# reuk/parallel-reverb-raytracer

Measured on AMD Instinct MI355X. Metric: ray_bounces_per_sec, higher is better.
Workload: dtype f32; 1 GPU; cathedral stand-in (Sibenik unavailable offline), 75252 triangles, 100000 rays/GPU x 128 bounces x 8 bands, 2 cardioid speakers, 44100 Hz, trim_predelay, output_mode all, histogram mode exact; triangles=75252, rays_per_gpu=100000, reflections=128, histogram_mode=exact: the reference's serial float sum over all impulses, bit for bit

## Files before the change

### parallel-reverb-raytracer_amd/csrc/ctx.h

```cpp
#pragma once

#include "../../include/rvb_capi.h"
#include "hip_owned.h"
#include "ir_state.h"
#include "kept_state.h"
#include "kernels.h"
#include "merged_state.h"
#include "source_state.h"
#include "trace_state.h"

#include <cmath>
#include <cstddef>
#include <cstring>
#include <memory>
#include <string>
#include <utility>
#include <vector>

#pragma GCC visibility push(hidden)

struct SceneStore {
    int device = 0;
    DevBuf nodes, tris, shade, corners, surfaces;
    ~SceneStore() { (void) hipSetDevice(device); }
// ... 350 lines not shown
    void end_timing(hipStream_t on = nullptr) { if (timing_open) (void) hipEventRecord(timings.back().stop, on ? on : stream.h); timing_open = false; }
    void reset_timings() { timings.clear(); events_used = 0; }
    void void_fetched_results() { trace.records_rewritten(); ir.drop_configuration(); }
    void void_trace() { trace.inputs_changed(); ir.drop_configuration(); merged.void_list(); }
};

int fail(rvb_ctx * ctx, int code, const std::string & what);
#define RVB_BIND(ctx) RVB_HIP(fail, ctx, hipSetDevice((ctx)->device))

inline const rvb_impulse * ir_diffuse(const rvb_ctx * ctx)
{
    return ctx->trace.impulses.as<rvb_impulse>() + ctx->trace.pair() * ctx->nrays * ctx->trace.nreflections();
}
struct IrCounts { uint64_t ndiffuse, nimages; };
inline IrCounts ir_counts(const rvb_ctx * ctx)
{
    return {(ctx->ir.which() & RVB_IR_DIFFUSE) ? ctx->nrays * ctx->trace.nreflections() : 0, (ctx->ir.which() & RVB_IR_IMAGES) ? ctx->ir.nimages() : 0};
}

inline uint64_t bins_for(float max_time, float predelay, float sample_rate)
{
    const float t = max_time > predelay ? max_time - predelay : 0.0f;
    return (uint64_t) (roundf(t * sample_rate) + 1);
}

inline int key_bits_for(uint64_t nbins)
{
    int bits = 1;
    while (bits < 32 && (1ull << bits) < nbins + 1)
        ++bits;
    return bits;
}

int fetch_small(rvb_ctx * ctx);
int reset_time_ranges(rvb_ctx * ctx, const TraceArgs & a);
int launch_images_beside(rvb_ctx * ctx, TraceArgs & a);
int launch_shadow_behind_images(rvb_ctx * ctx, const TraceArgs & a, const SourceShading & source, bool gains_stand = false);
int check_source_counts(rvb_ctx * ctx, const char * who, uint64_t npairs);
int apply_source_patterns(rvb_ctx * ctx, const TraceArgs & a, const SourceShading & source, bool gains_stand = false);
int download_surface_gradient(rvb_ctx * ctx, const float * d_out, rvb_surface * grad_surfaces, float grad_air[8]);

int merge_image_winners(const rvb_image_candidate * candidates, uint64_t ncandidates, bool have_direct, bool remove_direct, std::vector<uint32_t> & winners);
int ir_speaker_model(rvb_ctx * ctx, const float mic[3], const rvb_speaker * speakers, uint64_t nspeakers);
int ir_hrtf_model(rvb_ctx * ctx, const float mic[3], const float * table, const float facing[3], const float up[3]);
int ir_configure_refusals(rvb_ctx * ctx, int which);
int ir_configure_images(rvb_ctx * ctx, int which, const rvb_impulse * images, uint64_t nimages, bool gathered);
int ir_images_on_host(rvb_ctx * ctx);
int upload_hrtf_table(rvb_ctx * ctx, const float * table, int first_ear, int ears);
AttenuationModel hrtf_model(const rvb_ctx * ctx, const float mic[3], const float facing[3], const float up[3]);

bool own_sort_enabled();
int own_sort(rvb_ctx * ctx, const uint32_t * keys, uint32_t value_base, uint64_t n, int begin_bit, int end_bit,
             uint32_t * keys_out, uint32_t * values_out, bool want_keys);
int ensure_sort_buffers(rvb_ctx * ctx, uint64_t n);
int sort_and_bin(rvb_ctx * ctx, uint64_t n, uint64_t nkeys, int key_bits, bool may_sort_own);

#pragma GCC visibility pop
```

### parallel-reverb-raytracer_amd/csrc/exact_kernels.hip

```cpp
#include "attenuation.h"

#define SUM_UNROLL 4
#define RVB_HRTF_SUM_THREADS 256
#define WIDE_BINS 32
#define WIDE_MAX_WAVES 4

namespace {

__global__ __launch_bounds__(256) void bin_keys_kernel(ModelDev m, uint32_t ch, const rvb_impulse * __restrict__ in, uint64_t n,
                                                       uint64_t index_base, float predelay, float sample_rate, uint32_t sentinel,
                                                       uint32_t * __restrict__ keys, uint32_t * __restrict__ values)
{
    for (uint64_t i = (uint64_t) blockIdx.x * blockDim.x + threadIdx.x; i < n; i += (uint64_t) gridDim.x * blockDim.x) {
        const float4 * r = reinterpret_cast<const float4 *>(in + i);
        const float4 v0 = r[0], v1 = r[1], p = r[2];
        const float time = r[3].x;
        const bool nonzero = ANY_VOLUME(v0, v1);
        uint32_t key = sentinel;
        if (nonzero) key = min(time_bin(attenuated_time(m, ch, mk3(p.x, p.y, p.z), time), predelay, sample_rate), sentinel);
        keys[index_base + i] = key;
        values[index_base + i] = (uint32_t) (index_base + i);
    }
}

// ... 107 lines not shown
#pragma unroll 4
        for (uint32_t r = 0; r < LIVE_ROUNDS; ++r) {
            const uint64_t j = tile * RVB_LIVE_TILE + r * 64u + lane;
            const uint32_t key = j < n ? raw[j] : LIVE_DEAD;
            const bool live = key != LIVE_DEAD;
            const unsigned long long mask = __ballot(live);
            if (live) {
                const uint64_t to = at + lanes_below(mask);
                if (to < listed) {
                    keys[to] = key;
                    values[to] = (uint32_t) j;
                    if (HRTF) {
                        keys[listed + to] = raw[n + j];
                        values[listed + to] = (uint32_t) j;
                    }
                } else {
                    *overflow = 1u;
                }
            }
            at += (uint64_t) __popcll(mask);
        }
    }
    const uint64_t total = head->total < listed ? head->total : listed;
    for (uint64_t k = total + (uint64_t) blockIdx.x * blockDim.x + threadIdx.x; k < listed; k += (uint64_t) gridDim.x * blockDim.x) {
        keys[k] = nbins;
        values[k] = 0u;
        if (HRTF) {
            keys[listed + k] = 2u * nbins + 1u;
            values[listed + k] = 0u;
        }
    }
}

__global__ __launch_bounds__(256) void bin_starts_kernel(const uint32_t * __restrict__ keys, uint64_t n, uint64_t nbins, uint32_t * __restrict__ starts,
                                                         uint32_t * __restrict__ ends)
{
    for (uint64_t k = (uint64_t) blockIdx.x * blockDim.x + threadIdx.x; k < n; k += (uint64_t) gridDim.x * blockDim.x) {
        const uint32_t key = keys[k];
        if (key >= nbins)
            continue;
        if (k == 0 || keys[k - 1] != key)
            starts[key] = (uint32_t) k;
        if (k + 1 == n || keys[k + 1] != key)
            ends[key] = (uint32_t) (k + 1);
    }
}

template <bool HRTF, int NCH>
__global__ __launch_bounds__(64) void ordered_sum_kernel(ModelDev m, uint32_t first_channel, const rvb_impulse * __restrict__ diffuse,
                                                         uint64_t ndiffuse, const rvb_impulse * __restrict__ images,
                                                         const uint32_t * __restrict__ values,
                                                         const uint32_t * __restrict__ starts, const uint32_t * __restrict__ ends,
                                                         uint64_t nbins, uint64_t bin_begin, uint64_t bin_end, float * __restrict__ hist)
{
    const uint64_t t = (uint64_t) blockIdx.x * blockDim.x + threadIdx.x;
    const uint64_t bin = bin_begin + (t >> 1);
    const uint32_t half = (uint32_t) t & 1u;
    if (bin >= bin_end)
        return;
    const uint64_t lo = starts[bin];
    if (lo == 0xFFFFFFFFull)
        return;
    float sum[NCH][4];
#pragma unroll
    for (int c = 0; c < NCH; ++c)
#pragma unroll
        for (int b = 0; b < 4; ++b)
            sum[c][b] = hist[hist_row(first_channel + c, half, b, nbins) + bin];
    const uint64_t hi = ends[bin];
    for (uint64_t k = lo; k < hi; k += SUM_UNROLL) {
        float4 v[SUM_UNROLL], p[SUM_UNROLL];
        gather_records<SUM_UNROLL>(values, k, lo, hi, diffuse, ndiffuse, images, half, v, p);
#pragma unroll
        for (int u = 0; u < SUM_UNROLL; ++u) {
            if (k + u >= hi) break;
            const float vol[4] = {v[u].x, v[u].y, v[u].z, v[u].w};
            const v3 pos = mk3(p[u].x, p[u].y, p[u].z);
            if (HRTF) {
                const float * tb = m.table + ((uint64_t) first_channel * RVB_HRTF_ROWS + (uint64_t) hrtf_row(m, pos)) * 8 + half * 4;
#pragma unroll
                for (int b = 0; b < 4; ++b) sum[0][b] += vol[b] * tb[b];
            } else {
#pragma unroll
                for (int c = 0; c < NCH; ++c) {
                    const float g = speaker_gain(m, first_channel + c, pos);
#pragma unroll
                    for (int b = 0; b < 4; ++b) sum[c][b] += vol[b] * g;
                }
            }
        }
    }
#pragma unroll
    for (int c = 0; c < NCH; ++c)
#pragma unroll
        for (int b = 0; b < 4; ++b)
            hist[hist_row(first_channel + c, half, b, nbins) + bin] = sum[c][b];
}

__global__ __launch_bounds__(RVB_HRTF_SUM_THREADS) void ordered_sum_hrtf_kernel(ModelDev m, const rvb_impulse * __restrict__ diffuse, uint64_t ndiffuse,
                                                              const rvb_impulse * __restrict__ images, const uint32_t * __restrict__ values,
                                                              const uint32_t * __restrict__ starts, const uint32_t * __restrict__ ends,
                                                              uint64_t nbins, uint64_t bin_begin, uint64_t bin_end, float * __restrict__ hist)
{
    const uint64_t t = (uint64_t) blockIdx.x * blockDim.x + threadIdx.x;
    const uint64_t slot = 2 * bin_begin + (t >> 1);
    const uint32_t half = (uint32_t) t & 1u;
    if (slot >= 2 * bin_end)
        return;
    const uint32_t ear = (uint32_t) slot & 1u;
    const uint64_t bin = slot >> 1;
    const uint64_t key = (uint64_t) ear * (nbins + 1) + bin;
    const uint64_t lo = starts[key];
    if (lo == 0xFFFFFFFFull)
        return;
    float sum[4];
#pragma unroll
    for (int b = 0; b < 4; ++b)
        sum[b] = hist[((uint64_t) ear * 8 + half * 4 + b) * nbins + bin];
    const uint64_t hi = ends[key];
    const float * table = m.table + (uint64_t) ear * RVB_HRTF_ROWS * 8 + half * 4;
    for (uint64_t k = lo; k < hi; k += SUM_UNROLL) {
        float4 v[SUM_UNROLL], p[SUM_UNROLL];
        gather_records<SUM_UNROLL>(values, k, lo, hi, diffuse, ndiffuse, images, half, v, p);
#pragma unroll
        for (int u = 0; u < SUM_UNROLL; ++u) {
            if (k + u >= hi) break;
            const float4 tb = *reinterpret_cast<const float4 *>(table + (uint64_t) hrtf_row_quad(m, mk3(p[u].x, p[u].y, p[u].z), half) * 8);
            sum[0] += v[u].x * tb.x;
            sum[1] += v[u].y * tb.y;
// ... 100 lines not shown
        const float4 * r = reinterpret_cast<const float4 *>(in + values[k]);
        const float4 v0 = r[0], v1 = r[1];
        sum[0] += v0.x; sum[1] += v0.y; sum[2] += v0.z; sum[3] += v0.w;
        sum[4] += v1.x; sum[5] += v1.y; sum[6] += v1.z; sum[7] += v1.w;
    }
    for (int b = 0; b < 8; ++b)
        out[(uint64_t) b * nbins + bin] = sum[b];
}

bool fold_range(uint64_t nbins, uint64_t bin_begin, uint64_t & bin_end)
{
    bin_end = std::min(bin_end, nbins);
    return bin_begin < bin_end;
}

}

void rvb_launch_bin_keys(const AttenuationModel & m, uint32_t channel, const rvb_impulse * in, uint64_t n, uint64_t index_base,
                         float predelay, float sample_rate, uint32_t sentinel, uint32_t * keys, uint32_t * values, hipStream_t s)
{
    if (n == 0) return;
    hipLaunchKernelGGL(bin_keys_kernel, dim3(stream_blocks(n, 256)), dim3(256), 0, s, make_model(m), channel, in, n,
                       index_base, predelay, sample_rate, sentinel, keys, values);
}

void rvb_launch_bin_keys_hrtf(const AttenuationModel & m, const rvb_impulse * in, uint64_t count, uint64_t index_base, uint64_t n,
                              float predelay, float sample_rate, uint32_t nbins, uint32_t * keys, uint32_t * values, hipStream_t s)
{
    if (count == 0) return;
    hipLaunchKernelGGL(bin_keys_hrtf_kernel, dim3(stream_blocks(count, 256)), dim3(256), 0, s, make_model(m), in, count, index_base, n,
                       predelay, sample_rate, nbins, keys, values);
}

void rvb_launch_bin_starts(const uint32_t * sorted_keys, uint64_t n, uint64_t nbins, uint32_t * starts, uint32_t * ends, hipStream_t s)
{
    if (n == 0) return;
    hipLaunchKernelGGL(bin_starts_kernel, dim3(stream_blocks(n, 256)), dim3(256), 0, s, sorted_keys, n, nbins, starts, ends);
}

size_t rvb_live_scratch_bytes(uint64_t n)
{
    return sizeof(LiveHeader) + (size_t) ((n + RVB_LIVE_TILE - 1) / RVB_LIVE_TILE) * sizeof(uint32_t);
}

void rvb_launch_live_list(const AttenuationModel & m, const rvb_impulse * diffuse, uint64_t ndiffuse, const rvb_impulse * images, uint64_t n,
                          float predelay, float sample_rate, uint32_t nbins, uint64_t listed, uint32_t * raw, void * scratch,
                          uint32_t * keys, uint32_t * values, uint32_t * overflow, hipStream_t s)
{
    if (n == 0) return;
    LiveHeader * head = static_cast<LiveHeader *>(scratch);
    uint32_t * tiles = reinterpret_cast<uint32_t *>(head + 1);
    const uint64_t ntiles = (n + RVB_LIVE_TILE - 1) / RVB_LIVE_TILE;
    const dim3 grid(stream_blocks(ntiles, LIVE_WAVES)), block(64 * LIVE_WAVES);
    const ModelDev md = make_model(m);
    if (m.hrtf) {
        hipLaunchKernelGGL(live_keys_kernel<true>, grid, block, 0, s, md, diffuse, ndiffuse, images, n, predelay, sample_rate, nbins, raw, tiles);
        hipLaunchKernelGGL(live_offsets_kernel, dim3(1), dim3(LIVE_OFFSET_THREADS), 0, s, tiles, ntiles, head);
        hipLaunchKernelGGL(live_compact_kernel<true>, grid, block, 0, s, raw, n, tiles, head, listed, nbins, keys, values, overflow);
    } else {
        hipLaunchKernelGGL(live_keys_kernel<false>, grid, block, 0, s, md, diffuse, ndiffuse, images, n, predelay, sample_rate, nbins, raw, tiles);
        hipLaunchKernelGGL(live_offsets_kernel, dim3(1), dim3(LIVE_OFFSET_THREADS), 0, s, tiles, ntiles, head);
        hipLaunchKernelGGL(live_compact_kernel<false>, grid, block, 0, s, raw, n, tiles, head, listed, nbins, keys, values, overflow);
    }
}

void rvb_launch_ordered_sum(const AttenuationModel & m, uint32_t first_channel, uint32_t nchannels, const rvb_impulse * diffuse,
                            uint64_t ndiffuse, const rvb_impulse * images,
                            const uint32_t * sorted_values, const uint32_t * starts, const uint32_t * ends, uint64_t n,
                            uint64_t nbins, float * hist, hipStream_t s, uint64_t bin_begin, uint64_t bin_end)
{
    if (!fold_range(nbins, bin_begin, bin_end) || n == 0) return;
    const dim3 grid((unsigned) ((2 * (bin_end - bin_begin) + 63) / 64)), block(64);
    const ModelDev md = make_model(m);
#define RVB_SUM(HRTF, NCH) hipLaunchKernelGGL((ordered_sum_kernel<HRTF, NCH>), grid, block, 0, s, md, first_channel, diffuse, ndiffuse, \
                                              images, sorted_values, starts, ends, nbins, bin_begin, bin_end, hist)
    if (m.hrtf) { RVB_SUM(true, 1); return; }
    switch (nchannels) {
    case 1: RVB_SUM(false, 1); break;
    case 2: RVB_SUM(false, 2); break;
    case 3: RVB_SUM(false, 3); break;
    case 4: RVB_SUM(false, 4); break;
    default:
        for (uint32_t c = 0; c < nchannels; c += 4) {
            const uint32_t k = nchannels - c < 4 ? nchannels - c : 4;
            rvb_launch_ordered_sum(m, first_channel + c, k, diffuse, ndiffuse, images, sorted_values, starts, ends, n, nbins, hist, s, bin_begin, bin_end);
        }
    }
#undef RVB_SUM
}

void rvb_launch_ordered_sum_hrtf(const AttenuationModel & m, const rvb_impulse * diffuse, uint64_t ndiffuse, const rvb_impulse * images,
                                 const uint32_t * sorted_values, const uint32_t * starts, const uint32_t * ends, uint64_t nbins, float * hist,
                                 hipStream_t s, uint64_t bin_begin, uint64_t bin_end)
{
    if (!fold_range(nbins, bin_begin, bin_end)) return;
    const dim3 grid((unsigned) ((4 * (bin_end - bin_begin) + RVB_HRTF_SUM_THREADS - 1) / RVB_HRTF_SUM_THREADS));
    hipLaunchKernelGGL(ordered_sum_hrtf_kernel, grid, dim3(RVB_HRTF_SUM_THREADS), 0, s, make_model(m), diffuse, ndiffuse,
                       images, sorted_values, starts, ends, nbins, bin_begin, bin_end, hist);
}

void rvb_make_speaker_table(const rvb_speaker * speakers, uint64_t nspeakers, float4 * table)
{
    for (uint64_t i = 0; i < nspeakers; ++i)
        table[i] = speaker_device_form(speakers[i]);
}

void rvb_launch_ordered_sum_wide(const AttenuationModel & m, const rvb_impulse * diffuse, uint64_t ndiffuse, const rvb_impulse * images,
                                 const uint32_t * sorted_values, const uint32_t * starts, const uint32_t * ends, uint64_t n,
                                 uint64_t nbins, float * hist, hipStream_t s, uint64_t bin_begin, uint64_t bin_end)
{
    if (!fold_range(nbins, bin_begin, bin_end) || n == 0 || m.nchannels == 0 || !m.speaker_table) return;
    const uint32_t per_wave = wide_channels_per_wave(m.nchannels);
    const uint32_t waves = (m.nchannels + per_wave - 1) / per_wave;
    const dim3 grid((unsigned) ((bin_end - bin_begin + WIDE_BINS - 1) / WIDE_BINS)), block(64 * waves);
    const v3 mic = mk3(m.mic[0], m.mic[1], m.mic[2]);
    if (per_wave == 12)
        hipLaunchKernelGGL(ordered_sum_wide_kernel<12>, grid, block, 0, s, mic, m.speaker_table, m.nchannels, diffuse, ndiffuse, images,
                           sorted_values, starts, ends, nbins, bin_begin, bin_end, hist);
// ... 20 lines not shown
```

### parallel-reverb-raytracer_amd/csrc/ir.hip

```cpp
#include "bin_blocks.h"
#include "ctx.h"

#include <algorithm>
#include <cstdlib>
#include <cstring>

int upload_hrtf_table(rvb_ctx * ctx, const float * table, int first_ear, int ears)
{
    const size_t rows = RVB_HRTF_ROWS - 1;
    std::vector<float> padded((size_t) 2 * RVB_HRTF_ROWS * 8, 0.0f);
    for (int e = 0; e < ears; ++e)
        std::memcpy(padded.data() + (size_t) (first_ear + e) * RVB_HRTF_ROWS * 8, table + (size_t) e * rows * 8, rows * 8 * sizeof(float));
    RVB_HIP(fail, ctx, ctx->ir.hrtf_table.ensure(padded.size() * sizeof(float)));
    RVB_HIP(fail, ctx, hipMemcpy(ctx->ir.hrtf_table.p, padded.data(), padded.size() * sizeof(float), hipMemcpyHostToDevice));
    return RVB_OK;
}

AttenuationModel hrtf_model(const rvb_ctx * ctx, const float mic[3], const float facing[3], const float up[3])
{
    AttenuationModel m;
    m.hrtf = 1;
    m.nchannels = 2;
    m.hrtf_table = ctx->ir.hrtf_table.as<const float>();
    for (int i = 0; i < 3; ++i) { m.mic[i] = mic[i]; m.facing[i] = facing[i]; m.up[i] = up[i]; }
// ... 102 lines not shown
    in.ndiffuse = count.ndiffuse;
    in.nimages = count.nimages;
    in.n = in.ndiffuse + in.nimages;
    if (in.n >= (1ull << 31)) return fail(ctx, RVB_ERR_CAPACITY, "rvb_ir_accumulate: too many impulses for exact mode");
    if (nbins >= 0x7FFFFFF0ull) return fail(ctx, RVB_ERR_CAPACITY, "rvb_ir_accumulate: too many bins for exact mode");
    in.listed = in.n;
    return ensure_sort_buffers(ctx, lists * in.n);
}

int live_list(rvb_ctx * ctx, ExactList & in, float predelay, float sample_rate, uint64_t nbins)
{
    in.compacted = true;
    in.count_valid = ctx->trace.live_count_holds();
    if (in.count_valid && in.ndiffuse) {
        const int rc = fetch_small(ctx);
        if (rc != RVB_OK) return rc;
        in.listed = std::min<uint64_t>(ctx->trace.live_count(), in.ndiffuse) + in.nimages;
    }
    RVB_HIP(fail, ctx, ctx->sort.live.ensure(rvb_live_scratch_bytes(in.n)));
    rvb_launch_live_list(ctx->ir.model, ir_diffuse(ctx), in.ndiffuse, ctx->ir.images.as<rvb_impulse>(), in.n, predelay, sample_rate, (uint32_t) nbins,
                         in.listed, ctx->sort.keys_b.as<uint32_t>(), ctx->sort.live.p, ctx->sort.keys_a.as<uint32_t>(), ctx->sort.vals_a.as<uint32_t>(),
                         &ctx->trace.host->live_overflow, ctx->stream);
    return RVB_OK;
}

int exact_list(rvb_ctx * ctx, const ExactList & in, uint32_t channel, float predelay, float sample_rate, uint64_t nbins, bool may_sort_own)
{
    uint32_t * keys = ctx->sort.keys_a.as<uint32_t>(), * values = ctx->sort.vals_a.as<uint32_t>();
    rvb_launch_bin_keys(ctx->ir.model, channel, ir_diffuse(ctx), in.ndiffuse, 0, predelay, sample_rate, (uint32_t) nbins, keys, values, ctx->stream);
    rvb_launch_bin_keys(ctx->ir.model, channel, ctx->ir.images.as<rvb_impulse>(), in.nimages, in.ndiffuse, predelay, sample_rate, (uint32_t) nbins, keys, values, ctx->stream);
    return sort_and_bin(ctx, in.n, nbins, key_bits_for(nbins), may_sort_own);
}

int exact_prepare(rvb_ctx * ctx, float predelay, float sample_rate, uint64_t nbins)
{
    const AttenuationModel & m = ctx->ir.model;
    ExactList in;
    int rc = exact_begin(ctx, nbins, m.hrtf ? 2 : 1, in);
    if (rc != RVB_OK) return rc;
    if (m.hrtf) {
        const uint64_t nkeys = 2 * (nbins + 1);
        if ((rc = live_list(ctx, in, predelay, sample_rate, nbins)) == RVB_OK) rc = sort_and_bin(ctx, 2 * in.listed, nkeys, key_bits_for(nkeys - 1), false);
    } else if (own_sort_enabled()) {
        rc = exact_list(ctx, in, 0, predelay, sample_rate, nbins, true);
    } else {
        if ((rc = live_list(ctx, in, predelay, sample_rate, nbins)) == RVB_OK) rc = sort_and_bin(ctx, in.listed, nbins, key_bits_for(nbins), false);
    }
    if (rc != RVB_OK) return rc;
    RVB_HIP(fail, ctx, hipGetLastError());
    in.hrtf_combined = m.hrtf != 0;
    ctx->ir.exact_prepared(in);
    return RVB_OK;
}

int exact_fold(rvb_ctx * ctx, uint64_t b0, uint64_t b1, float * hist)
{
    const AttenuationModel & m = ctx->ir.model;
    const ExactList & e = ctx->ir.exact();
    if (!ctx->ir.prepared()) return fail(ctx, RVB_ERR_STATE, "rvb_ir_exact_fold: rvb_ir_exact_prepare first (and nothing that reuses the sort buffers in between)");
    if (b1 > e.nbins) b1 = e.nbins;
    if (e.hrtf_combined) {
        const uint64_t nkeys = 2 * (e.nbins + 1);
        rvb_launch_ordered_sum_hrtf(m, ir_diffuse(ctx), e.ndiffuse, ctx->ir.images.as<rvb_impulse>(), ctx->sort.vals_b.as<uint32_t>(),
                                    ctx->sort.bin_starts.as<uint32_t>(), ctx->sort.bin_starts.as<uint32_t>() + nkeys, e.nbins, hist, ctx->stream, b0, b1);
    } else if (m.nchannels > 8) {
        rvb_launch_ordered_sum_wide(m, ir_diffuse(ctx), e.ndiffuse, ctx->ir.images.as<rvb_impulse>(), ctx->sort.vals_b.as<uint32_t>(),
                                    ctx->sort.bin_starts.as<uint32_t>(), ctx->sort.bin_starts.as<uint32_t>() + e.nbins, e.listed, e.nbins, hist, ctx->stream, b0, b1);
    } else {
        rvb_launch_ordered_sum(m, 0, m.nchannels, ir_diffuse(ctx), e.ndiffuse, ctx->ir.images.as<rvb_impulse>(), ctx->sort.vals_b.as<uint32_t>(),
                               ctx->sort.bin_starts.as<uint32_t>(), ctx->sort.bin_starts.as<uint32_t>() + e.nbins, e.listed, e.nbins, hist, ctx->stream, b0, b1);
    }
    RVB_HIP(fail, ctx, hipGetLastError());
    return RVB_OK;
}

int exact_split_ears(rvb_ctx * ctx, float predelay, float sample_rate, uint64_t nbins, float * hist)
{
    const AttenuationModel & m = ctx->ir.model;
    ExactList in;
    int rc = exact_begin(ctx, nbins, 1, in);
    for (uint32_t ch = 0; rc == RVB_OK && ch < m.nchannels; ++ch) {
        if ((rc = exact_list(ctx, in, ch, predelay, sample_rate, nbins, false)) != RVB_OK) break;
        rvb_launch_ordered_sum(m, ch, 1u, ir_diffuse(ctx), in.ndiffuse, ctx->ir.images.as<rvb_impulse>(), ctx->sort.vals_b.as<uint32_t>(),
                               ctx->sort.bin_starts.as<uint32_t>(), ctx->sort.bin_starts.as<uint32_t>() + nbins, in.n, nbins, hist, ctx->stream);
    }
    return rc;
}

int export_bin_range(rvb_ctx * ctx, float * pinned_dst, const float * hist, uint64_t rows, uint64_t nbins, uint64_t b0, uint64_t b1)
{
    if (b1 <= b0) return RVB_OK;
    RVB_HIP(fail, ctx, hipEventRecord(ctx->export_ready, ctx->stream));
    RVB_HIP(fail, ctx, hipStreamWaitEvent(ctx->export_stream, ctx->export_ready, 0));
    if (b0 == 0 && b1 == nbins) {
        RVB_HIP(fail, ctx, hipMemcpyAsync(pinned_dst, hist, rows * nbins * sizeof(float), hipMemcpyDeviceToHost, ctx->export_stream));
    } else {
        RVB_HIP(fail, ctx, hipMemcpy2DAsync(pinned_dst + b0, nbins * sizeof(float), hist + b0, nbins * sizeof(float), (b1 - b0) * sizeof(float), rows,
                                            hipMemcpyDeviceToHost, ctx->export_stream));
    }
    return RVB_OK;
}

int ir_accumulate_impl(rvb_ctx * ctx, float predelay, float sample_rate, uint64_t nbins, int mode, void * d_histogram,
// ... 217 lines not shown
```

### parallel-reverb-raytracer_amd/csrc/ir_state.h

```cpp
#pragma once

#include <cstdint>

#pragma GCC visibility push(hidden)

struct FlattenQuery {
    const void * host = nullptr;
    uint64_t n = 0, bins = 0;
    float sample_rate = 0.0f;
};

struct ExactList {
    bool hrtf_combined = false;
    uint64_t nbins = 0, n = 0, ndiffuse = 0, nimages = 0;
    uint64_t listed = 0;
    bool count_valid = false, compacted = false;
};

class IrState {
public:
    enum Tenant { NOTHING, FLATTEN_QUERY, EXACT_LIST };

    bool configured() const { return configured_; }
    int which() const { return which_; }
    uint64_t nimages() const { return nimages_; }
    bool from_merged_list() const { return from_merged_list_; }
    bool host_images_stale() const { return host_images_stale_; }
    bool range_pending() const { return range_pending_; }
    int table_ears() const { return table_ears_; }
    Tenant tenant() const { return tenant_; }
    const FlattenQuery & query() const { return query_; }
    const ExactList & exact() const { return exact_; }
    bool resident(const void * in, uint64_t n, float sample_rate) const
    {
        return tenant_ == FLATTEN_QUERY && in != nullptr && query_.host == in && query_.n == n && query_.sample_rate == sample_rate;
    }
    bool prepared() const { return tenant_ == EXACT_LIST; }
    bool ever_listed() const { return ever_listed_; }
    bool prepared_for(uint64_t nbins) const { return prepared() && exact_.nbins == nbins; }

    void configure(int which, uint64_t nimages, bool gathered)
    {
        which_ = which;
        nimages_ = nimages;
        from_merged_list_ = host_images_stale_ = gathered;
        configured_ = true;
        void_exact_list();
        range_pending_ = false;
    }
// ... 37 lines not shown
```

### parallel-reverb-raytracer_amd/csrc/kernels.h

```cpp
#pragma once

#include <hip/hip_runtime.h>
#include <stdint.h>

#include "../../include/rvb_capi.h"
#include "../../include/rvb_capi_live.h"
#include "../../include/rvb_capi_window.h"
#include "bvh.h"

struct SceneDev {
    const BvhNode * nodes = nullptr;
    const BvhTri * tris = nullptr;
    const TriShade * shade = nullptr;
    const TriCorners * corners = nullptr;
    const rvb_surface * surfaces = nullptr;
    uint32_t ntris = 0;
    float cull_abs = 0.0f;
    float cull_rel = 0.0f;
    unsigned long long * stamps = nullptr;
};

struct ImageItem { uint32_t ray, index; };
struct TraceArgs {
    SceneDev scene;
// ... 135 lines not shown
                                 DecayParamsRow * rows, double * loss_rows, hipStream_t s);
void rvb_launch_decay_params_adjoint_sums(const float * curve, uint64_t nrows, uint64_t nbins, const DecayParamsRow * rows, double * tiles, hipStream_t s);
void rvb_launch_decay_params_adjoint_carry(uint64_t nrows, uint64_t nbins, double * tiles, hipStream_t s);
void rvb_launch_decay_params_adjoint_scan(const float * hist, const float * curve, uint64_t nrows, uint64_t nbins, const DecayParamsRow * rows,
                                          const double * tiles, float * weights, hipStream_t s);
size_t rvb_group_records_temp_bytes(uint64_t n);
hipError_t rvb_group_records(void * temp, size_t temp_bytes, const uint32_t * keys, uint32_t * keys_scratch, uint32_t * order,
                             uint64_t n, uint32_t first_record, int begin_bit, int end_bit, hipStream_t s);
hipError_t rvb_group_records16(void * temp, size_t temp_bytes, const uint16_t * keys, uint16_t * keys_scratch, uint32_t * order,
                               uint64_t n, uint32_t first_record, int begin_bit, int end_bit, hipStream_t s);

struct AttenuationModel {
    int hrtf = 0;
    uint32_t nchannels = 0;
    float mic[3] = {0, 0, 0};
    rvb_speaker speakers[8] = {};
    const float4 * speaker_table = nullptr;
    const float * hrtf_table = nullptr;
    float facing[3] = {0, 0, 0}, up[3] = {0, 0, 0};
};

void rvb_launch_attenuate(const AttenuationModel & m, uint32_t channel, const rvb_impulse * in, uint64_t n,
                          rvb_attenuated_impulse * out, hipStream_t s);
void rvb_launch_time_range(const AttenuationModel & m, const rvb_impulse * in, uint64_t n, uint32_t * range, hipStream_t s);
void rvb_launch_histogram_fast(const AttenuationModel & m, const rvb_impulse * in, uint64_t n, float predelay,
                               float sample_rate, uint64_t nbins, float * acc, hipStream_t s);
void rvb_launch_histogram_transpose(const float * acc, float * hist, uint32_t nchannels, uint64_t nbins, hipStream_t s);
void rvb_launch_add(float * acc, const float * x, uint64_t n, hipStream_t s);
void rvb_launch_bin_keys(const AttenuationModel & m, uint32_t channel, const rvb_impulse * in, uint64_t n, uint64_t index_base,
                         float predelay, float sample_rate, uint32_t sentinel, uint32_t * keys, uint32_t * values, hipStream_t s);
void rvb_launch_ordered_sum(const AttenuationModel & m, uint32_t first_channel, uint32_t nchannels, const rvb_impulse * diffuse,
                            uint64_t ndiffuse, const rvb_impulse * images,
                            const uint32_t * sorted_values, const uint32_t * starts, const uint32_t * ends, uint64_t n,
                            uint64_t nbins, float * hist, hipStream_t s, uint64_t bin_begin = 0, uint64_t bin_end = ~0ull);
void rvb_make_speaker_table(const rvb_speaker * speakers, uint64_t nspeakers, float4 * table);
void rvb_launch_ordered_sum_wide(const AttenuationModel & m, const rvb_impulse * diffuse, uint64_t ndiffuse, const rvb_impulse * images,
                                 const uint32_t * sorted_values, const uint32_t * starts, const uint32_t * ends, uint64_t n,
                                 uint64_t nbins, float * hist, hipStream_t s, uint64_t bin_begin = 0, uint64_t bin_end = ~0ull);
void rvb_launch_bin_keys_hrtf(const AttenuationModel & m, const rvb_impulse * in, uint64_t count, uint64_t index_base, uint64_t n,
                              float predelay, float sample_rate, uint32_t nbins, uint32_t * keys, uint32_t * values, hipStream_t s);
void rvb_launch_ordered_sum_hrtf(const AttenuationModel & m, const rvb_impulse * diffuse, uint64_t ndiffuse, const rvb_impulse * images,
                                 const uint32_t * sorted_values, const uint32_t * starts, const uint32_t * ends, uint64_t nbins, float * hist,
                                 hipStream_t s, uint64_t bin_begin = 0, uint64_t bin_end = ~0ull);
size_t rvb_live_scratch_bytes(uint64_t n);
void rvb_launch_live_list(const AttenuationModel & m, const rvb_impulse * diffuse, uint64_t ndiffuse, const rvb_impulse * images, uint64_t n,
                          float predelay, float sample_rate, uint32_t nbins, uint64_t listed, uint32_t * raw, void * scratch,
                          uint32_t * keys, uint32_t * values, uint32_t * overflow, hipStream_t s);
void rvb_launch_bin_starts(const uint32_t * sorted_keys, uint64_t n, uint64_t nbins, uint32_t * starts, uint32_t * ends, hipStream_t s);
void rvb_launch_flat_keys(const rvb_attenuated_impulse * in, uint64_t n, float sample_rate, uint32_t * keys, uint32_t * values,
                          uint32_t * max_time_bits, hipStream_t s);
void rvb_launch_flat_ordered_sum(const rvb_attenuated_impulse * in, const uint32_t * sorted_keys, const uint32_t * sorted_values,
                                 const uint32_t * starts, uint64_t n, uint64_t nbins, float * out, hipStream_t s);
void rvb_launch_fix_predelay(rvb_attenuated_impulse * a, uint64_t n, float seconds, hipStream_t s);
size_t rvb_radix_sort_temp_bytes(uint64_t n);
hipError_t rvb_radix_sort_pairs(void * temp, size_t temp_bytes, const uint32_t * keys, const uint32_t * values, uint32_t value_base,
                                uint32_t * keys_a, uint32_t * values_a, uint32_t * keys_b, uint32_t * values_b, uint64_t n,
                                int begin_bit, int end_bit, bool want_keys, const uint32_t ** keys_sorted, const uint32_t ** values_sorted,
                                hipStream_t s);
size_t rvb_sort_temp_bytes(uint64_t n);
void rvb_sort_pairs(void * temp, size_t temp_bytes, const uint32_t * keys_in, uint32_t * keys_out,
                    const uint32_t * values_in, uint32_t * values_out, uint64_t n, int key_bits, hipStream_t s);
struct WindowWeights { float w[8]; };
size_t rvb_window_scratch_bytes(uint64_t n);
rvb_window_entry * rvb_window_scratch_entries(void * scratch);
const void * rvb_window_scratch_state(const void * scratch);
hipError_t rvb_launch_window_begin(void * scratch, hipStream_t s);
void rvb_launch_window_score(const rvb_impulse * in, uint64_t n, float t_begin, float t_end, const WindowWeights & weights, void * scratch, hipStream_t s);
void rvb_launch_window_pass(uint32_t pass, uint64_t n, uint64_t max_entries, void * scratch, hipStream_t s);
void rvb_launch_window_gather(uint64_t n, void * scratch, hipStream_t s);
void rvb_launch_window_sort(const rvb_impulse * in, void * scratch, rvb_window_entry * entries, hipStream_t s);
void rvb_launch_window_paths(const rvb_impulse * in, const uint2 * listen, uint32_t nreflections, uint64_t max_paths, uint64_t max_hits,
                             const void * scratch, rvb_window_path * paths, rvb_window_hit * hits, hipStream_t s);
```

### parallel-reverb-raytracer_amd/csrc/rocprim_sort.hip

```cpp
#include <algorithm>

#include "kernels.h"

#include <rocprim/device/device_radix_sort.hpp>
#include <rocprim/iterator/counting_iterator.hpp>

size_t rvb_sort_temp_bytes(uint64_t n)
{
    size_t bytes = 0;
    (void) rocprim::radix_sort_pairs(nullptr, bytes, (const uint32_t *) nullptr, (uint32_t *) nullptr,
                              (const uint32_t *) nullptr, (uint32_t *) nullptr, (size_t) n, 0, 32, (hipStream_t) 0);
    return bytes;
}

void rvb_sort_pairs(void * temp, size_t temp_bytes, const uint32_t * keys_in, uint32_t * keys_out,
                    const uint32_t * values_in, uint32_t * values_out, uint64_t n, int key_bits, hipStream_t s)
{
    if (n == 0) return;
    (void) rocprim::radix_sort_pairs(temp, temp_bytes, keys_in, keys_out, values_in, values_out, (size_t) n, 0, (unsigned) key_bits, s);
}

size_t rvb_group_records_temp_bytes(uint64_t n)
{
    size_t bytes16 = 0;
    (void) rocprim::radix_sort_pairs(nullptr, bytes16, (const uint16_t *) nullptr, (uint16_t *) nullptr,
                                     rocprim::counting_iterator<uint32_t>(0), (uint32_t *) nullptr, (size_t) n, 0, 16, (hipStream_t) 0);
    size_t bytes = 0;
    const hipError_t e = rocprim::radix_sort_pairs(nullptr, bytes, (const uint32_t *) nullptr, (uint32_t *) nullptr,
                                                   rocprim::counting_iterator<uint32_t>(0), (uint32_t *) nullptr, (size_t) n, 0, 32,
                                                   (hipStream_t) 0);
    (void) hipGetLastError();
    return e == hipSuccess ? std::max(bytes, bytes16) : 0;
}

hipError_t rvb_group_records(void * temp, size_t temp_bytes, const uint32_t * keys, uint32_t * keys_scratch, uint32_t * order,
                             uint64_t n, uint32_t first_record, int begin_bit, int end_bit, hipStream_t s)
{
    if (n == 0) return hipSuccess;
    return rocprim::radix_sort_pairs(temp, temp_bytes, keys, keys_scratch, rocprim::counting_iterator<uint32_t>(first_record), order,
                                     (size_t) n, (unsigned) begin_bit, (unsigned) end_bit, s);
}

hipError_t rvb_group_records16(void * temp, size_t temp_bytes, const uint16_t * keys, uint16_t * keys_scratch, uint32_t * order,
                               uint64_t n, uint32_t first_record, int begin_bit, int end_bit, hipStream_t s)
{
    if (n == 0) return hipSuccess;
    return rocprim::radix_sort_pairs(temp, temp_bytes, keys, keys_scratch, rocprim::counting_iterator<uint32_t>(first_record), order,
                                     (size_t) n, (unsigned) begin_bit, (unsigned) end_bit, s);
}
```

### parallel-reverb-raytracer_amd/csrc/sort.hip

```cpp
#include "ctx.h"

#include <cstdlib>
#include <cstring>

bool own_sort_enabled()
{
    static const bool own = getenv("RVB_SORT") && std::strcmp(getenv("RVB_SORT"), "own") == 0;
    return own;
}

int own_sort(rvb_ctx * ctx, const uint32_t * keys, uint32_t value_base, uint64_t n, int begin_bit, int end_bit,
             uint32_t * keys_out, uint32_t * values_out, bool want_keys)
{
    if (n == 0 || end_bit <= begin_bit) return RVB_OK;
    const int passes = (end_bit - begin_bit + 7) / 8;
    RVB_HIP(fail, ctx, ctx->sort.own_temp.ensure(rvb_radix_sort_temp_bytes(n)));
    uint32_t * tmp_k = nullptr, * tmp_v = nullptr;
    if (passes > 1) {
        RVB_HIP(fail, ctx, ctx->sort.own_keys.ensure(n * 4));
        RVB_HIP(fail, ctx, ctx->sort.own_values.ensure(n * 4));
        tmp_k = ctx->sort.own_keys.as<uint32_t>();
        tmp_v = ctx->sort.own_values.as<uint32_t>();
    }
    const bool last_in_b = ((passes - 1) & 1) != 0;
    uint32_t * ka = last_in_b ? tmp_k : keys_out, * va = last_in_b ? tmp_v : values_out;
    uint32_t * kb = last_in_b ? keys_out : tmp_k, * vb = last_in_b ? values_out : tmp_v;
    const uint32_t * ks = nullptr, * vs = nullptr;
    RVB_HIP(fail, ctx, rvb_radix_sort_pairs(ctx->sort.own_temp.p, ctx->sort.own_temp.cap, keys, nullptr, value_base, ka, va, kb, vb, n,
                                            begin_bit, end_bit, want_keys, &ks, &vs, ctx->stream));
    if (vs != values_out || (want_keys && ks != keys_out)) return fail(ctx, RVB_ERR_HIP, "internal error: radix sort result in the wrong buffer");
    return RVB_OK;
}

int ensure_sort_buffers(rvb_ctx * ctx, uint64_t n)
{
    SortBuffers & b = ctx->sort;
    ctx->ir.sort_buffers_claimed();
    RVB_HIP(fail, ctx, b.keys_a.ensure(n * 4));
    RVB_HIP(fail, ctx, b.keys_b.ensure(n * 4));
    RVB_HIP(fail, ctx, b.vals_a.ensure(n * 4));
    RVB_HIP(fail, ctx, b.vals_b.ensure(n * 4));
    RVB_HIP(fail, ctx, b.temp.ensure(rvb_sort_temp_bytes(n)));
    return RVB_OK;
}

int sort_and_bin(rvb_ctx * ctx, uint64_t n, uint64_t nkeys, int key_bits, bool may_sort_own)
{
    SortBuffers & b = ctx->sort;
    RVB_HIP(fail, ctx, b.bin_starts.ensure(nkeys * 8));
    uint32_t * starts = b.bin_starts.as<uint32_t>();
    if (may_sort_own && own_sort_enabled()) {
        const int rc = own_sort(ctx, b.keys_a.as<uint32_t>(), 0u, n, 0, key_bits, b.keys_b.as<uint32_t>(), b.vals_b.as<uint32_t>(), true);
        if (rc != RVB_OK) return rc;
    } else {
        rvb_sort_pairs(b.temp.p, b.temp.cap, b.keys_a.as<uint32_t>(), b.keys_b.as<uint32_t>(),
                       b.vals_a.as<uint32_t>(), b.vals_b.as<uint32_t>(), n, key_bits, ctx->stream);
    }
    RVB_HIP(fail, ctx, hipMemsetAsync(starts, 0xFF, nkeys * 4, ctx->stream));
    rvb_launch_bin_starts(b.keys_b.as<uint32_t>(), n, nkeys, starts, starts + nkeys, ctx->stream);
    return RVB_OK;
}
```

Before: 3.191 billion ray-bounces/s.

## Sort exact-histogram keys only on coarse bits and sum runs of 32 bins per wave

The radix sort of impulse keys now skips the low 5 bits, so it orders entries by groups of 32 bins instead of by exact bin, which needs fewer sort passes. A new coarse ordered-sum kernel gives each 32-bin group to one 64-lane wave. Each chunk of entries is staged in shared memory, and a ballot per bin lets the lanes assigned to that bin accumulate the matching entries in index order, which keeps the serial float sum order. The per-run start and end offsets come from atomics. This adds ballot and shared-memory work inside the summation, and it relies on a stable sort to keep the bit-exact order.

```diff
diff --git a/parallel-reverb-raytracer_amd/csrc/ctx.h b/parallel-reverb-raytracer_amd/csrc/ctx.h
--- a/parallel-reverb-raytracer_amd/csrc/ctx.h
+++ b/parallel-reverb-raytracer_amd/csrc/ctx.h
@@ -406,6 +406,11 @@
     return bits;
 }
 
+inline uint64_t coarse_keys(uint64_t nkeys, int shift)
+{
+    return (nkeys + (1ull << shift) - 1) >> shift;
+}
+
 int fetch_small(rvb_ctx * ctx);
 int reset_time_ranges(rvb_ctx * ctx, const TraceArgs & a);
 int launch_images_beside(rvb_ctx * ctx, TraceArgs & a);
@@ -427,6 +432,6 @@
 int own_sort(rvb_ctx * ctx, const uint32_t * keys, uint32_t value_base, uint64_t n, int begin_bit, int end_bit,
              uint32_t * keys_out, uint32_t * values_out, bool want_keys);
 int ensure_sort_buffers(rvb_ctx * ctx, uint64_t n);
-int sort_and_bin(rvb_ctx * ctx, uint64_t n, uint64_t nkeys, int key_bits, bool may_sort_own);
+int sort_and_bin(rvb_ctx * ctx, uint64_t n, uint64_t nkeys, int key_bits, bool may_sort_own, int coarse_shift = 0);
 
 #pragma GCC visibility pop
diff --git a/parallel-reverb-raytracer_amd/csrc/exact_kernels.hip b/parallel-reverb-raytracer_amd/csrc/exact_kernels.hip
--- a/parallel-reverb-raytracer_amd/csrc/exact_kernels.hip
+++ b/parallel-reverb-raytracer_amd/csrc/exact_kernels.hip
@@ -163,13 +163,22 @@
     }
 }
 
-__global__ __launch_bounds__(256) void bin_starts_kernel(const uint32_t * __restrict__ keys, uint64_t n, uint64_t nbins, uint32_t * __restrict__ starts,
-                                                         uint32_t * __restrict__ ends)
+__global__ __launch_bounds__(256) void bin_starts_kernel(const uint32_t * __restrict__ keys, uint64_t n, uint64_t nbins, uint32_t shift,
+                                                         uint32_t * __restrict__ starts, uint32_t * __restrict__ ends)
 {
     for (uint64_t k = (uint64_t) blockIdx.x * blockDim.x + threadIdx.x; k < n; k += (uint64_t) gridDim.x * blockDim.x) {
         const uint32_t key = keys[k];
         if (key >= nbins)
             continue;
+        if (shift) {
+            const uint32_t run = key >> shift;
+            const uint32_t before = k == 0 ? 0xFFFFFFFFu : keys[k - 1], after = k + 1 == n ? 0xFFFFFFFFu : keys[k + 1];
+            if (before >= nbins || (before >> shift) != run)
+                atomicMin(starts + run, (uint32_t) k);
+            if (after >= nbins || (after >> shift) != run)
+                atomicMax(ends + run, (uint32_t) (k + 1));
+            continue;
+        }
         if (k == 0 || keys[k - 1] != key)
             starts[key] = (uint32_t) k;
         if (k + 1 == n || keys[k + 1] != key)
@@ -226,6 +235,98 @@
 #pragma unroll
         for (int b = 0; b < 4; ++b)
             hist[hist_row(first_channel + c, half, b, nbins) + bin] = sum[c][b];
+}
+
+#define COARSE_CHUNK 64
+static_assert(COARSE_CHUNK == 64 && RVB_COARSE_BINS * 2 == 64, "an entry per lane, a lane pair per bin");
+template <int NCH>
+__global__ __launch_bounds__(64)
+void ordered_sum_coarse_kernel(ModelDev m, uint32_t first_channel, const rvb_impulse * __restrict__ diffuse, uint64_t ndiffuse,
+                               const rvb_impulse * __restrict__ images, const uint32_t * __restrict__ keys,
+                               const uint32_t * __restrict__ values, const uint32_t * __restrict__ starts,
+                               const uint32_t * __restrict__ ends, uint64_t nbins, uint64_t bin_begin, uint64_t bin_end,
+                               float * __restrict__ hist)
+{
+    __shared__ float4 s_vol[COARSE_CHUNK][2];
+    __shared__ float s_gain[COARSE_CHUNK][NCH];
+    const uint32_t lane = threadIdx.x;
+    const uint64_t coarse = (bin_begin >> RVB_COARSE_SHIFT) + blockIdx.x;
+    const uint64_t lo = starts[coarse];
+    if (lo == 0xFFFFFFFFull)
+        return;
+    const uint64_t hi = ends[coarse];
+    const uint32_t half = lane & 1u, pair = lane >> 1;
+    const uint32_t first_bin = (uint32_t) (coarse << RVB_COARSE_SHIFT);
+    const uint64_t bin = (uint64_t) first_bin + pair;
+    const bool mine = bin >= bin_begin && bin < bin_end;
+    float sum[NCH][4];
+#pragma unroll
+    for (int c = 0; c < NCH; ++c)
+#pragma unroll
+        for (int b = 0; b < 4; ++b)
+            sum[c][b] = mine ? hist[hist_row(first_channel + c, half, b, nbins) + bin] : 0.0f;
+    bool touched = false;
+
+    uint32_t key, value, next_key, next_value;
+    float4 v0, v1, p;
+#define COARSE_ENTRY(K, KEY, VALUE) do { const uint64_t at_ = (K) + lane; const bool in_ = at_ < hi; \
+                                         KEY = in_ ? keys[at_] : 0xFFFFFFFFu; VALUE = in_ ? values[at_] : 0u; } while (0)
+#define COARSE_TAKEN(KEY) ((KEY) >= bin_begin && (KEY) < bin_end)
+#define COARSE_GATHER() do { if (COARSE_TAKEN(key)) { \
+                                 const float4 * r_ = reinterpret_cast<const float4 *>(value < ndiffuse ? diffuse + value : images + (value - ndiffuse)); \
+                                 v0 = r_[0]; v1 = r_[1]; p = r_[2]; } } while (0)
+    v0 = v1 = p = make_float4(0.0f, 0.0f, 0.0f, 0.0f);
+    COARSE_ENTRY(lo, key, value);
+    COARSE_GATHER();
+    COARSE_ENTRY(lo + COARSE_CHUNK, next_key, next_value);
+    for (uint64_t k = lo; k < hi; k += COARSE_CHUNK) {
+        const bool taken = COARSE_TAKEN(key);
+        const uint32_t slot = taken ? key - first_bin : 0xFFFFFFFFu;
+        if (taken) {
+            s_vol[lane][0] = v0;
+            s_vol[lane][1] = v1;
+            const v3 pos = mk3(p.x, p.y, p.z);
+#pragma unroll
+            for (int c = 0; c < NCH; ++c)
+                s_gain[lane][c] = speaker_gain(m, first_channel + c, pos);
+        }
+        key = next_key;
+        value = next_value;
+        COARSE_GATHER();
+        COARSE_ENTRY(k + 2 * COARSE_CHUNK, next_key, next_value);
+        __syncthreads();
+        unsigned long long todo = 0;
+#pragma unroll
+        for (uint32_t q = 0; q < RVB_COARSE_BINS; ++q) {
+            const unsigned long long holders = __ballot(slot == q);
+            if (pair == q) todo = holders;
+        }
+        if (!mine) todo = 0;
+        while (todo) {
+            const uint32_t e = (uint32_t) __ffsll((long long) todo) - 1u;
+            todo &= todo - 1;
+            const float4 v = s_vol[e][half];
+            const float vol[4] = {v.x, v.y, v.z, v.w};
+#pragma unroll
+            for (int c = 0; c < NCH; ++c) {
+                const float g = s_gain[e][c];
+#pragma unroll
+                for (int b = 0; b < 4; ++b) sum[c][b] += vol[b] * g;
+            }
+            touched = true;
+        }
+        __syncthreads();
+    }
+#undef COARSE_ENTRY
+#undef COARSE_TAKEN
+#undef COARSE_GATHER
+    if (touched) {
+#pragma unroll
+        for (int c = 0; c < NCH; ++c)
+#pragma unroll
+            for (int b = 0; b < 4; ++b)
+                hist[hist_row(first_channel + c, half, b, nbins) + bin] = sum[c][b];
+    }
 }
 
 __global__ __launch_bounds__(RVB_HRTF_SUM_THREADS) void ordered_sum_hrtf_kernel(ModelDev m, const rvb_impulse * __restrict__ diffuse, uint64_t ndiffuse,
@@ -392,10 +493,10 @@
                        predelay, sample_rate, nbins, keys, values);
 }
 
-void rvb_launch_bin_starts(const uint32_t * sorted_keys, uint64_t n, uint64_t nbins, uint32_t * starts, uint32_t * ends, hipStream_t s)
+void rvb_launch_bin_starts(const uint32_t * sorted_keys, uint64_t n, uint64_t nbins, uint32_t * starts, uint32_t * ends, hipStream_t s, int shift)
 {
     if (n == 0) return;
-    hipLaunchKernelGGL(bin_starts_kernel, dim3(stream_blocks(n, 256)), dim3(256), 0, s, sorted_keys, n, nbins, starts, ends);
+    hipLaunchKernelGGL(bin_starts_kernel, dim3(stream_blocks(n, 256)), dim3(256), 0, s, sorted_keys, n, nbins, (uint32_t) shift, starts, ends);
 }
 
 size_t rvb_live_scratch_bytes(uint64_t n)
@@ -427,13 +528,17 @@
 void rvb_launch_ordered_sum(const AttenuationModel & m, uint32_t first_channel, uint32_t nchannels, const rvb_impulse * diffuse,
                             uint64_t ndiffuse, const rvb_impulse * images,
                             const uint32_t * sorted_values, const uint32_t * starts, const uint32_t * ends, uint64_t n,
-                            uint64_t nbins, float * hist, hipStream_t s, uint64_t bin_begin, uint64_t bin_end)
+                            uint64_t nbins, float * hist, hipStream_t s, uint64_t bin_begin, uint64_t bin_end, const uint32_t * coarse_keys)
 {
     if (!fold_range(nbins, bin_begin, bin_end) || n == 0) return;
-    const dim3 grid((unsigned) ((2 * (bin_end - bin_begin) + 63) / 64)), block(64);
+    const bool coarse = coarse_keys != nullptr && !m.hrtf;
+    const dim3 grid(coarse ? (unsigned) (((bin_end - 1) >> RVB_COARSE_SHIFT) - (bin_begin >> RVB_COARSE_SHIFT) + 1)
+                           : (unsigned) ((2 * (bin_end - bin_begin) + 63) / 64)), block(64);
     const ModelDev md = make_model(m);
-#define RVB_SUM(HRTF, NCH) hipLaunchKernelGGL((ordered_sum_kernel<HRTF, NCH>), grid, block, 0, s, md, first_channel, diffuse, ndiffuse, \
-                                              images, sorted_values, starts, ends, nbins, bin_begin, bin_end, hist)
+#define RVB_SUM(HRTF, NCH) do { if (coarse) hipLaunchKernelGGL((ordered_sum_coarse_kernel<NCH>), grid, block, 0, s, md, first_channel, diffuse, ndiffuse, \
+                                                               images, coarse_keys, sorted_values, starts, ends, nbins, bin_begin, bin_end, hist); \
+                                else hipLaunchKernelGGL((ordered_sum_kernel<HRTF, NCH>), grid, block, 0, s, md, first_channel, diffuse, ndiffuse, \
+                                                        images, sorted_values, starts, ends, nbins, bin_begin, bin_end, hist); } while (0)
     if (m.hrtf) { RVB_SUM(true, 1); return; }
     switch (nchannels) {
     case 1: RVB_SUM(false, 1); break;
@@ -443,7 +548,8 @@
     default:
         for (uint32_t c = 0; c < nchannels; c += 4) {
             const uint32_t k = nchannels - c < 4 ? nchannels - c : 4;
-            rvb_launch_ordered_sum(m, first_channel + c, k, diffuse, ndiffuse, images, sorted_values, starts, ends, n, nbins, hist, s, bin_begin, bin_end);
+            rvb_launch_ordered_sum(m, first_channel + c, k, diffuse, ndiffuse, images, sorted_values, starts, ends, n, nbins, hist, s, bin_begin, bin_end,
+                                   coarse_keys);
         }
     }
 #undef RVB_SUM
diff --git a/parallel-reverb-raytracer_amd/csrc/ir.hip b/parallel-reverb-raytracer_amd/csrc/ir.hip
--- a/parallel-reverb-raytracer_amd/csrc/ir.hip
+++ b/parallel-reverb-raytracer_amd/csrc/ir.hip
@@ -158,6 +158,12 @@
     return sort_and_bin(ctx, in.n, nbins, key_bits_for(nbins), may_sort_own);
 }
 
+bool coarse_list_enabled()
+{
+    static const bool on = !(getenv("RVB_EXACT_COARSE") && std::strcmp(getenv("RVB_EXACT_COARSE"), "0") == 0);
+    return on;
+}
+
 int exact_prepare(rvb_ctx * ctx, float predelay, float sample_rate, uint64_t nbins)
 {
     const AttenuationModel & m = ctx->ir.model;
@@ -170,7 +176,9 @@
     } else if (own_sort_enabled()) {
         rc = exact_list(ctx, in, 0, predelay, sample_rate, nbins, true);
     } else {
-        if ((rc = live_list(ctx, in, predelay, sample_rate, nbins)) == RVB_OK) rc = sort_and_bin(ctx, in.listed, nbins, key_bits_for(nbins), false);
+        in.coarse_shift = m.nchannels <= 8 && coarse_list_enabled() ? RVB_COARSE_SHIFT : 0;
+        if ((rc = live_list(ctx, in, predelay, sample_rate, nbins)) == RVB_OK)
+            rc = sort_and_bin(ctx, in.listed, nbins, key_bits_for(nbins), false, in.coarse_shift);
     }
     if (rc != RVB_OK) return rc;
     RVB_HIP(fail, ctx, hipGetLastError());
@@ -193,8 +201,10 @@
         rvb_launch_ordered_sum_wide(m, ir_diffuse(ctx), e.ndiffuse, ctx->ir.images.as<rvb_impulse>(), ctx->sort.vals_b.as<uint32_t>(),
                                     ctx->sort.bin_starts.as<uint32_t>(), ctx->sort.bin_starts.as<uint32_t>() + e.nbins, e.listed, e.nbins, hist, ctx->stream, b0, b1);
     } else {
+        const uint64_t nruns = coarse_keys(e.nbins, e.coarse_shift);
         rvb_launch_ordered_sum(m, 0, m.nchannels, ir_diffuse(ctx), e.ndiffuse, ctx->ir.images.as<rvb_impulse>(), ctx->sort.vals_b.as<uint32_t>(),
-                               ctx->sort.bin_starts.as<uint32_t>(), ctx->sort.bin_starts.as<uint32_t>() + e.nbins, e.listed, e.nbins, hist, ctx->stream, b0, b1);
+                               ctx->sort.bin_starts.as<uint32_t>(), ctx->sort.bin_starts.as<uint32_t>() + nruns, e.listed, e.nbins, hist, ctx->stream, b0, b1,
+                               e.coarse_shift ? ctx->sort.keys_b.as<uint32_t>() : nullptr);
     }
     RVB_HIP(fail, ctx, hipGetLastError());
     return RVB_OK;
diff --git a/parallel-reverb-raytracer_amd/csrc/ir_state.h b/parallel-reverb-raytracer_amd/csrc/ir_state.h
--- a/parallel-reverb-raytracer_amd/csrc/ir_state.h
+++ b/parallel-reverb-raytracer_amd/csrc/ir_state.h
@@ -15,6 +15,7 @@
     uint64_t nbins = 0, n = 0, ndiffuse = 0, nimages = 0;
     uint64_t listed = 0;
     bool count_valid = false, compacted = false;
+    int coarse_shift = 0;
 };
 
 class IrState {
diff --git a/parallel-reverb-raytracer_amd/csrc/kernels.h b/parallel-reverb-raytracer_amd/csrc/kernels.h
--- a/parallel-reverb-raytracer_amd/csrc/kernels.h
+++ b/parallel-reverb-raytracer_amd/csrc/kernels.h
@@ -191,7 +191,10 @@
 void rvb_launch_ordered_sum(const AttenuationModel & m, uint32_t first_channel, uint32_t nchannels, const rvb_impulse * diffuse,
                             uint64_t ndiffuse, const rvb_impulse * images,
                             const uint32_t * sorted_values, const uint32_t * starts, const uint32_t * ends, uint64_t n,
-                            uint64_t nbins, float * hist, hipStream_t s, uint64_t bin_begin = 0, uint64_t bin_end = ~0ull);
+                            uint64_t nbins, float * hist, hipStream_t s, uint64_t bin_begin = 0, uint64_t bin_end = ~0ull,
+                            const uint32_t * coarse_keys = nullptr);
+#define RVB_COARSE_SHIFT 5
+#define RVB_COARSE_BINS (1u << RVB_COARSE_SHIFT)
 void rvb_make_speaker_table(const rvb_speaker * speakers, uint64_t nspeakers, float4 * table);
 void rvb_launch_ordered_sum_wide(const AttenuationModel & m, const rvb_impulse * diffuse, uint64_t ndiffuse, const rvb_impulse * images,
                                  const uint32_t * sorted_values, const uint32_t * starts, const uint32_t * ends, uint64_t n,
@@ -205,7 +208,7 @@
 void rvb_launch_live_list(const AttenuationModel & m, const rvb_impulse * diffuse, uint64_t ndiffuse, const rvb_impulse * images, uint64_t n,
                           float predelay, float sample_rate, uint32_t nbins, uint64_t listed, uint32_t * raw, void * scratch,
                           uint32_t * keys, uint32_t * values, uint32_t * overflow, hipStream_t s);
-void rvb_launch_bin_starts(const uint32_t * sorted_keys, uint64_t n, uint64_t nbins, uint32_t * starts, uint32_t * ends, hipStream_t s);
+void rvb_launch_bin_starts(const uint32_t * sorted_keys, uint64_t n, uint64_t nbins, uint32_t * starts, uint32_t * ends, hipStream_t s, int shift = 0);
 void rvb_launch_flat_keys(const rvb_attenuated_impulse * in, uint64_t n, float sample_rate, uint32_t * keys, uint32_t * values,
                           uint32_t * max_time_bits, hipStream_t s);
 void rvb_launch_flat_ordered_sum(const rvb_attenuated_impulse * in, const uint32_t * sorted_keys, const uint32_t * sorted_values,
@@ -218,7 +221,7 @@
                                 hipStream_t s);
 size_t rvb_sort_temp_bytes(uint64_t n);
 void rvb_sort_pairs(void * temp, size_t temp_bytes, const uint32_t * keys_in, uint32_t * keys_out,
-                    const uint32_t * values_in, uint32_t * values_out, uint64_t n, int key_bits, hipStream_t s);
+                    const uint32_t * values_in, uint32_t * values_out, uint64_t n, int begin_bit, int key_bits, hipStream_t s);
 struct WindowWeights { float w[8]; };
 size_t rvb_window_scratch_bytes(uint64_t n);
 rvb_window_entry * rvb_window_scratch_entries(void * scratch);
diff --git a/parallel-reverb-raytracer_amd/csrc/rocprim_sort.hip b/parallel-reverb-raytracer_amd/csrc/rocprim_sort.hip
--- a/parallel-reverb-raytracer_amd/csrc/rocprim_sort.hip
+++ b/parallel-reverb-raytracer_amd/csrc/rocprim_sort.hip
@@ -14,10 +14,11 @@
 }
 
 void rvb_sort_pairs(void * temp, size_t temp_bytes, const uint32_t * keys_in, uint32_t * keys_out,
-                    const uint32_t * values_in, uint32_t * values_out, uint64_t n, int key_bits, hipStream_t s)
+                    const uint32_t * values_in, uint32_t * values_out, uint64_t n, int begin_bit, int key_bits, hipStream_t s)
 {
     if (n == 0) return;
-    (void) rocprim::radix_sort_pairs(temp, temp_bytes, keys_in, keys_out, values_in, values_out, (size_t) n, 0, (unsigned) key_bits, s);
+    (void) rocprim::radix_sort_pairs(temp, temp_bytes, keys_in, keys_out, values_in, values_out, (size_t) n, (unsigned) begin_bit,
+                                     (unsigned) key_bits, s);
 }
 
 size_t rvb_group_records_temp_bytes(uint64_t n)
diff --git a/parallel-reverb-raytracer_amd/csrc/sort.hip b/parallel-reverb-raytracer_amd/csrc/sort.hip
--- a/parallel-reverb-raytracer_amd/csrc/sort.hip
+++ b/parallel-reverb-raytracer_amd/csrc/sort.hip
@@ -44,19 +44,24 @@
     return RVB_OK;
 }
 
-int sort_and_bin(rvb_ctx * ctx, uint64_t n, uint64_t nkeys, int key_bits, bool may_sort_own)
+int sort_and_bin(rvb_ctx * ctx, uint64_t n, uint64_t nkeys, int key_bits, bool may_sort_own, int coarse_shift)
 {
     SortBuffers & b = ctx->sort;
-    RVB_HIP(fail, ctx, b.bin_starts.ensure(nkeys * 8));
+    const uint64_t nruns = coarse_keys(nkeys, coarse_shift);
+    RVB_HIP(fail, ctx, b.bin_starts.ensure(nruns * 8));
     uint32_t * starts = b.bin_starts.as<uint32_t>();
-    if (may_sort_own && own_sort_enabled()) {
+    if (coarse_shift > 0 && key_bits <= coarse_shift) {
+        RVB_HIP(fail, ctx, hipMemcpyAsync(b.keys_b.p, b.keys_a.p, n * 4, hipMemcpyDeviceToDevice, ctx->stream));
+        RVB_HIP(fail, ctx, hipMemcpyAsync(b.vals_b.p, b.vals_a.p, n * 4, hipMemcpyDeviceToDevice, ctx->stream));
+    } else if (coarse_shift == 0 && may_sort_own && own_sort_enabled()) {
         const int rc = own_sort(ctx, b.keys_a.as<uint32_t>(), 0u, n, 0, key_bits, b.keys_b.as<uint32_t>(), b.vals_b.as<uint32_t>(), true);
         if (rc != RVB_OK) return rc;
     } else {
         rvb_sort_pairs(b.temp.p, b.temp.cap, b.keys_a.as<uint32_t>(), b.keys_b.as<uint32_t>(),
-                       b.vals_a.as<uint32_t>(), b.vals_b.as<uint32_t>(), n, key_bits, ctx->stream);
+                       b.vals_a.as<uint32_t>(), b.vals_b.as<uint32_t>(), n, coarse_shift, key_bits, ctx->stream);
     }
-    RVB_HIP(fail, ctx, hipMemsetAsync(starts, 0xFF, nkeys * 4, ctx->stream));
-    rvb_launch_bin_starts(b.keys_b.as<uint32_t>(), n, nkeys, starts, starts + nkeys, ctx->stream);
+    RVB_HIP(fail, ctx, hipMemsetAsync(starts, 0xFF, nruns * 4, ctx->stream));
+    if (coarse_shift > 0) RVB_HIP(fail, ctx, hipMemsetAsync(starts + nruns, 0, nruns * 4, ctx->stream));
+    rvb_launch_bin_starts(b.keys_b.as<uint32_t>(), n, nkeys, starts, starts + nruns, ctx->stream, coarse_shift);
     return RVB_OK;
 }
```

Result: faster. 3.236 billion ray-bounces/s, median of 6 (+1.4%).
